# rhasspy/larynx

Measured on AMD Instinct MI355X. Metric: utterances_per_sec, higher is better.
Workload: dtype f32; 1 GPU; en-us ljspeech GlowTTS + hifi_gan 'high', batch=1, 120 phoneme ids per utterance (~623 frames = 7.24 s audio), seeded random weights, device RNG noise, fused one-call entry (mi355tts_synthesize), denoiser off (the Python API default); ids_per_utterance=120, parallelism=utterance-dp1, batch=1, calls_in_flight_per_gpu=8

## Files before the change

### larynx_amd/csrc/host_launch.h

```cpp
#pragma once

struct RowLen {
  const int* len;
  int len_const;
  template <class Args>
  void into(Args& a) const { a.len = len; a.len_const = len_const; }
};
static inline RowLen row_len(int B, int host_len, const int* dev_len, int mul = 1, int dev_const = 0) {
  if (B == 1 && host_len >= 0) return {nullptr, host_len * mul};
  return {dev_len, dev_const};
}

template <int K, int CI_C, int MB, int NB, int WN, int KS, int HALO, int EPI>
static void launch_conv_inst(ProfScope& ps, hipStream_t s, dim3 grid, const ConvArgs& a) {
  ps.kernel(KN_CONV_MFMA, a.rows);
  hipLaunchKernelGGL(HIP_KERNEL_NAME(conv_mfma_kernel<K, CI_C, MB, NB, WN, KS, HALO, EPI>), grid, dim3(64 * WN * KS), 0, s, a);
}

enum TileShape { TILE_SMALL = 0, TILE_W128 = 1, TILE_NB2 = 2, TILE_TINY = 3, TILE_LAST = 3, TILE_M128 = 4 };

static bool rb_plane_ok(const ConvArgs& a) { return (long long)a.Cin * a.x_ld < (1LL << 30); }

template <int K, int EPI>
static int launch_conv_k(ProfScope& ps, hipStream_t s, int MB, int shape, dim3 grid, const ConvArgs& a, bool rb_conv) {
  constexpr int HALO = conv_halo(K);
  constexpr int CI_SMALL = (K == 1) ? 64 : 32;
  constexpr bool PAIRED = (EPI == EPI_GATE || EPI == EPI_COUPLING);
  if (!halo_fits(K, a.dil, a.pad, HALO))
    return fail(MI355TTS_ERR_INVALID, "conv K=%d dilation=%d exceeds the staged halo", K, a.dil);
  if (a.x_ld % 4) return fail(MI355TTS_ERR_INVALID, "internal: activation row stride %d is not a multiple of 4", a.x_ld);
  if constexpr (EPI == EPI_LINEAR && K >= 3) {
    if (shape == TILE_M128) {
      ps.kernel(KN_CONV_M128, a.rows);
      hipLaunchKernelGGL(HIP_KERNEL_NAME(conv_mfma_kernel<K, 16, 1, 2, 1, 1, HALO, EPI, 4>), grid, dim3(256), 0, s, a);
      return 0;
    }
  }
  if constexpr (EPI == EPI_UPSAMPLE) {
    if (shape == TILE_M128) {
      if constexpr (K == 2) {
        if (rb_conv && a.Cin % 16 == 0 && !a.res && !a.accum && a.alpha == 1.0f && rb_plane_ok(a)) {
          if (a.x2 && a.x3) hipLaunchKernelGGL(HIP_KERNEL_NAME(rb_conv_kernel<2, 4, EPI_UPSAMPLE, true>), grid, dim3(256), 0, s, a);
          else if (!a.x2) hipLaunchKernelGGL(HIP_KERNEL_NAME(rb_conv_kernel<2, 4, EPI_UPSAMPLE, false>), grid, dim3(256), 0, s, a);
          if ((a.x2 && a.x3) || !a.x2) {
            ps.kernel(KN_RB_CONV, a.rows);
            return 0;
          }
        }
      }
      ps.kernel(KN_CONV_M128, a.rows);
      hipLaunchKernelGGL(HIP_KERNEL_NAME(conv_mfma_kernel<K, 16, 1, 2, 1, 1, HALO, EPI, 4>), grid, dim3(256), 0, s, a);
      return 0;
    }
  }
  if (shape == TILE_M128) return fail(MI355TTS_ERR_INVALID, "internal: the 128-row tile is a ResBlock conv / upsampler shape");
  if (MB == 1) {
    if (shape == TILE_TINY) launch_conv_inst<K, 64, 1, 1, 1, 8, HALO, EPI>(ps, s, grid, a);
    else if (shape == TILE_SMALL) launch_conv_inst<K, CI_SMALL, 1, 1, 2, 4, HALO, EPI>(ps, s, grid, a);
    else if (shape == TILE_W128) launch_conv_inst<K, 32, 1, 2, 2, 4, HALO, EPI>(ps, s, grid, a);
    else launch_conv_inst<K, 16, 1, 2, 4, 2, HALO, EPI>(ps, s, grid, a);
    return 0;
  }
  if constexpr (!PAIRED) {
    if (shape == TILE_TINY) launch_conv_inst<K, 64, 2, 1, 1, 8, HALO, EPI>(ps, s, grid, a);
    else if (shape == TILE_SMALL) launch_conv_inst<K, CI_SMALL, 2, 1, 2, 4, HALO, EPI>(ps, s, grid, a);
    else if (shape == TILE_W128) return fail(MI355TTS_ERR_INVALID, "internal: the 128-column tile is one m-tile high");
    else launch_conv_inst<K, 16, 2, 2, 4, 2, HALO, EPI>(ps, s, grid, a);
    return 0;
  }
  return fail(MI355TTS_ERR_INVALID, "paired epilogues run on 32-row tiles (MB == 1)");
}

struct ConvPlan {
  ConvArgs a;
  int K = 0, MB = 1, shape = TILE_TINY, epi = EPI_LINEAR, cls = 0;
  dim3 grid;
  double flop = 0;
  bool empty = true;
  int bf16 = 0;
  int n_max = 0;
  bool pinned = false;
};

enum Bf16Cfg {
  BF_A = 0,
  BF_B = 1,
  BF_C = 2,
  BF_D = 3,
  BF_K = 4,
};
struct Bf16Tile {
  int NB, WM, WN, KS;
};
constexpr Bf16Tile BF16_TILES[5] = {{4, 4, 1, 1}, {1, 4, 1, 1}, {2, 2, 2, 1}, {1, 1, 4, 1}, {4, 4, 1, 2}};
template <class F>
static bool bf16_dispatch(int cfg, int bf16, F&& f) {
  return switch_const<BF_A, BF_B, BF_C, BF_D, BF_K>(cfg, [&](auto c) {
    if (bf16 == 3) f(c, int_c<3>{});
    else f(c, int_c<1>{});
  });
}
template <int K, int EPI>
static int launch_bf16_k(int cfg, int bf16, dim3 grid, hipStream_t s, const ConvArgs& a) {
  const bool known = bf16_dispatch(cfg, bf16, [&](auto c, auto terms) {
    constexpr Bf16Tile t = BF16_TILES[decltype(c)::value];
    hipLaunchKernelGGL(HIP_KERNEL_NAME(conv_bf16_kernel<K, 1, t.NB, t.WM, t.WN, conv_halo(K), decltype(terms)::value, t.KS, EPI>), grid,
                       dim3(64 * t.WM * t.WN * t.KS), 0, s, a);
  });
  return known ? 0 : fail(MI355TTS_ERR_INVALID, "internal: bf16 tile %d", cfg);
}

static int plan_conv(const CallOptions& o, const DevConv& c, ConvArgs a, int epi, int B, int n_max, int cls, int min_tiles, int host_len, ConvPlan* out,
                     int precision = 0) {
  out->empty = true;
  out->bf16 = 0;
  if (n_max <= 0 || B <= 0) return 0;
  auto side = [&](const int*& len, int& len_const, int mul) {
    if (!len) return;
    const RowLen r = row_len(B, host_len, len, mul, len_const);
    len = r.len; len_const = r.len_const;
// ... 8 lines not shown
  a.Cin = c.Cin;
  a.rows = c.rows;
  const bool half_on = (precision == MI355TTS_PRECISION_BF16X3 || precision == MI355TTS_PRECISION_BF16) && c.w16 && (a.x_ld % 4) == 0;
  const bool bf_linear = half_on && epi == EPI_LINEAR && !a.x2 && !a.y2 && a.split >= c.rows && a.out_act == ACT_NONE &&
                         (c.K == 3 || c.K == 5 || c.K == 7 || c.K == 11) && halo_fits(c.K, a.dil, a.pad, conv_halo(c.K));
  const bool bf_ups = half_on && !o.env.bf16_ups_off && epi == EPI_UPSAMPLE && c.K == 2 && halo_fits(2, a.dil, a.pad, conv_halo(2));
  if (bf_linear || bf_ups) {
    a.w16 = c.w16;
    a.nslab = c.nslab16;
    a.rows_major = 0;
    if (epi == EPI_UPSAMPLE) {
      const double w_bytes = (double)c.mtiles16 * c.nslab16 * c.K * 2048.0, x_bytes = (double)c.Cin * (double)n_max * 4.0 * B;
      a.rows_major = (w_bytes > x_bytes && x_bytes < 3.0e6 && c.mtiles16 >= 32) ? 1 : 0;
    }
    int cfg, rows_t, cols_t;
    if (c.mtiles16 % 4 == 0) {
      const long long tiles_a = (long long)((n_max + 127) / 128) * (c.mtiles16 / 4) * B;
      cfg = tiles_a >= 256 ? BF_A : (o.env.bf_k_off ? BF_B : BF_K);
      rows_t = 128;
      cols_t = cfg == BF_B ? 32 : 128;
    } else if (c.mtiles16 == 2) {
      cfg = BF_C;
      rows_t = 64;
      cols_t = 128;
    } else {
      cfg = BF_D;
      rows_t = 32;
      cols_t = 128;
    }
    out->a = a;
    out->K = c.K;
    out->MB = 1;
    out->shape = cfg;
    out->epi = epi;
    out->cls = cls;
    out->bf16 = precision == MI355TTS_PRECISION_BF16 ? 1 : 3;
    out->n_max = n_max;
    out->pinned = false;
    out->grid = dim3((n_max + cols_t - 1) / cols_t, (c.mtiles16 * 32) / rows_t, B);
    out->flop = 2.0 * (double)c.Cout * c.Cin * (epi == EPI_UPSAMPLE ? c.K * a.up : c.K) * (double)n_max * B;
    out->empty = false;
    return 0;
  }
  int MB = c.MB;
  int ytiles = c.mtiles / MB;
  const int rows32 = (c.rows + 31) / 32;
  auto tiles = [&](int width) { return (long long)((n_max + width - 1) / width) * (width == 128 ? rows32 : ytiles) * B; };
  const long long want = min_tiles;
  int shape = TILE_TINY;
  if (tiles(256) >= want) shape = TILE_NB2;
  else if (tiles(128) >= want) shape = TILE_W128;
  else if (tiles(64) >= want) shape = TILE_SMALL;
  bool pinned = false;
  {
    int f = o.env.force_tile;
    if (o.env.force_tile_dynamic != KNOB_UNSET) f = o.env.force_tile_dynamic;
    if (o.pin_tile >= 0) f = o.pin_tile;
    if (f >= TILE_SMALL && f <= TILE_LAST) {
      shape = f;
      pinned = true;
    }
  }
  if (shape == TILE_TINY && MB == 2 && (epi == EPI_LINEAR || epi == EPI_UPSAMPLE) && tiles(32) < 256) {
    MB = 1;
    ytiles = rows32;
  }
  {
    if (o.env.ups64 && !pinned && epi == EPI_UPSAMPLE && c.MB == 2 && rows32 == 2 && shape == TILE_W128 && tiles(64) >= 256) shape = TILE_SMALL;
  }
  if (shape == TILE_W128 && MB == 2) {
    MB = 1;
    ytiles = rows32;
  }
  {
    const bool resblock_ok = epi == EPI_LINEAR && cls == KC_RESBLOCK && c.K >= 3;
    const bool upsample_ok = epi == EPI_UPSAMPLE && !o.env.m128_ups_off && c.K >= 1 && c.K <= 3;
    if (!o.env.m128_off && !pinned && (resblock_ok || upsample_ok) && rows32 % 4 == 0 && c.rows == rows32 * 32 &&
        (long long)((n_max + 127) / 128) * (rows32 / 4) * B >= o.env.m128_min_tiles) {
      shape = TILE_M128;
      MB = 1;
      ytiles = rows32 / 4;
    }
  }
  const int T_T = shape == TILE_TINY ? 32 : (shape == TILE_SMALL || shape == TILE_M128) ? 64 : (shape == TILE_NB2 ? 256 : 128);
  {
    const double w_bytes = (double)c.mtiles * c.noct * c.K * 1024.0;
    const double x_bytes = (double)c.Cin * (double)n_max * 4.0 * B;
    a.rows_major = (w_bytes > x_bytes && x_bytes < 3.0e6 && ytiles >= 8) ? 1 : 0;
  }
  out->a = a;
  out->K = c.K;
  out->MB = MB;
  out->shape = shape;
  out->epi = epi;
  out->cls = cls;
  out->n_max = n_max;
  out->pinned = pinned;
  out->grid = dim3((n_max + T_T - 1) / T_T, ytiles, B);
  out->flop = 2.0 * (double)c.Cout * c.Cin * (epi == EPI_UPSAMPLE ? c.K * a.up : c.K) * (double)n_max * B;
  out->empty = false;
  return 0;
}

template <int EPI, int... Ks>
static int launch_conv_taps(ProfScope& ps, const ConvPlan& p, const char* unsupported, hipStream_t s, bool rb_conv) {
  int rc = 0;
  if (!switch_const<Ks...>(p.K, [&](auto k) { rc = launch_conv_k<decltype(k)::value, EPI>(ps, s, p.MB, p.shape, p.grid, p.a, rb_conv); }))
    rc = fail(MI355TTS_ERR_INVALID, unsupported, p.K);
  return rc;
}
static int run_plan(mi355tts_ctx* ctx, Worker* w, const ConvPlan& p, hipStream_t stream = nullptr) {
  if (p.empty) return 0;
  hipStream_t s = stream ? stream : w->stream;
  ProfScope ps(ctx, w, p.cls, p.flop, s);
  const bool rb_conv = w->opt.rb_conv && !w->opt.env.rb_conv_off;
  if (p.bf16) {
    ps.kernel(KN_CONV_BF16, p.a.rows);
    if (p.epi == EPI_UPSAMPLE) {
      if (p.K != 2) return fail(MI355TTS_ERR_INVALID, "bf16 upsampler needs two taps");
      return launch_bf16_k<2, EPI_UPSAMPLE>(p.shape, p.bf16, p.grid, s, p.a);
    }
    int rc = 0;
    if (!switch_const<3, 5, 7, 11>(p.K, [&](auto k) { rc = launch_bf16_k<decltype(k)::value, EPI_LINEAR>(p.shape, p.bf16, p.grid, s, p.a); }))
      rc = fail(MI355TTS_ERR_INVALID, "unsupported conv kernel size %d in bf16 mode", p.K);
    return rc;
  }
  if (p.epi == EPI_LINEAR) return launch_conv_taps<EPI_LINEAR, 1, 3, 5, 7, 11>(ps, p, "unsupported conv kernel size %d", s, rb_conv);
  if (p.epi == EPI_GATE) return launch_conv_taps<EPI_GATE, 3, 5>(ps, p, "unsupported WaveNet kernel size %d", s, rb_conv);
  if (p.epi == EPI_COUPLING) return launch_conv_taps<EPI_COUPLING, 1>(ps, p, "coupling conv must be 1x1", s, rb_conv);
  return launch_conv_taps<EPI_UPSAMPLE, 1, 2, 3>(ps, p, "unsupported upsample taps %d", s, rb_conv);
}

static int launch_conv(mi355tts_ctx* ctx, Worker* w, const DevConv& c, ConvArgs a, int epi, int B, int n_max, int cls,
                       hipStream_t stream = nullptr, int min_tiles = 1024, int host_len = -1, int precision = 0) {
  ConvPlan p;
  CHECK(plan_conv(w->opt, c, a, epi, B, n_max, cls, min_tiles, host_len, &p, precision));
  return run_plan(ctx, w, p, stream);
}

struct GroupTile {
  int shape, MB, CI_C, MBT, NB, WN, KS, WM;
};
constexpr GroupTile GROUP_TILES[6] = {{TILE_M128, 0, 16, 1, 2, 1, 1, 4}, {TILE_NB2, 2, 16, 2, 2, 4, 2, 1},  {TILE_W128, 1, 32, 1, 2, 2, 4, 1},
                                      {TILE_SMALL, 2, 32, 2, 1, 2, 4, 1}, {TILE_TINY, 1, 64, 1, 1, 1, 8, 1}, {TILE_TINY, 2, 64, 2, 1, 1, 8, 1}};
static int group_tile(int shape, int MB) {
  for (int i = 0; i < 6; ++i)
    if (GROUP_TILES[i].shape == shape && (GROUP_TILES[i].MB == MB || GROUP_TILES[i].MB == 0)) return i;
  return -1;
}
template <int K0, int K1, int K2>
static void launch_group_k(ProfScope& ps, hipStream_t s, int tile, dim3 grid, const ConvGroupArgs& g) {
  ps.kernel(KN_CONV_GROUP, g.c[0].rows);
  switch_const<0, 1, 2, 3, 4, 5>(tile, [&](auto i) {
    constexpr GroupTile t = GROUP_TILES[decltype(i)::value];
    hipLaunchKernelGGL(HIP_KERNEL_NAME(conv_group_kernel<K0, K1, K2, t.CI_C, t.MBT, t.NB, t.WN, t.KS, conv_halo(K0), conv_halo(K1), conv_halo(K2), t.WM>),
                       grid, dim3(64 * t.WM * t.WN * t.KS), 0, s, g);
  });
}
static bool rb_member_ok(const ConvArgs& a, int K) {
  const int halo = K == 11 ? RbCfg<11>::HALO : K == 7 ? RbCfg<7>::HALO : RbCfg<3>::HALO;
  return !a.x2 && !a.x3 && a.bias && a.alpha == 1.0f && !a.accum && a.out_act == ACT_NONE && a.split >= a.rows && !a.y2 &&
         a.rows % 128 == 0 && halo_fits(K, a.dil, a.pad, halo) && rb_plane_ok(a);
}

static void promote_group_plans(const CallOptions& o, ConvPlan* const* plans, int n) {
  if (n != 3 || o.env.group_promote_off || !o.group_promote) return;
  int K[3], tiles[3];
// ... 402 lines not shown
```

### larynx_amd/csrc/host_options.h

```cpp
#pragma once

constexpr int KNOB_UNSET = INT_MIN;
enum KnobWhen { PROCESS, CALL };
#define MI355TTS_ENV_KNOBS(X)                                                                                                       \
  X(sync_mode, "MI355TTS_SYNC_MODE", int, 3, PROCESS, "initial g_sync_mode: 0 hipStreamSynchronize, 1 blocking event, 2 query + sleep, 3 adaptive") \
  X(queue_policy, "MI355TTS_QUEUE_POLICY", int, 0, PROCESS, "acquire_worker: 1 = an idle hardware queue first, else the BUSIEST one (probe)") \
  X(queue_probe_off, "MI355TTS_NO_QUEUE_PROBE", bool, false, PROCESS, "no measurement of which worker streams share a hardware queue") \
  X(call_coalesce_off, "MI355TTS_NO_CALL_COALESCE", bool, false, PROCESS, "every call runs alone whatever option call_coalesce says") \
  X(selfcheck_off, "MI355TTS_NO_SELFCHECK", bool, false, PROCESS, "no dispatch-order self-check (looked at again when the check would run)") \
  X(rb_tiles, "MI355TTS_RB_TILES", int, 0, PROCESS, "workgroup target per ResBlock conv launch (<= 0: 1024)")                       \
  X(glow_tiles, "MI355TTS_GLOW_TILES", int, 0, PROCESS, "workgroup target per GlowTTS conv launch (<= 0: 1024)")                    \
  X(force_tile, "MI355TTS_FORCE_TILE", int, -1, PROCESS, "pins plan_conv's tile shape (0 .. 3): sweeps")                            \
  X(ups64, "MI355TTS_UPS64", bool, true, PROCESS, "64-row upsamplers on the 64 x 64 tile; 0 = plan_conv's shape rule (A/B runs)")   \
  X(m128_off, "MI355TTS_NO_M128", bool, false, PROCESS, "no 128-row tile at all")                                                    \
  X(m128_ups_off, "MI355TTS_NO_M128_UPS", bool, false, PROCESS, "no 128-row tile for the upsamplers")                                \
  X(rb_conv_off, "MI355TTS_NO_RB_CONV", bool, false, PROCESS, "grouped 128-row launches and upsamplers on the chunked tile, as option rb_conv = 0") \
  X(group_off, "MI355TTS_NO_GROUP", bool, false, PROCESS, "no grouped launches: neither run_group nor run_pair_group")               \
  X(group_promote_off, "MI355TTS_NO_GROUP_PROMOTE", bool, false, PROCESS, "batch-1 ResBlock steps stay on the tiles plan_conv chose") \
  X(snake_off, "MI355TTS_NO_SNAKE", bool, false, PROCESS, "grouped launches keep the longest-first order")                           \
  X(pair_fusion_off, "MI355TTS_NO_PAIR_FUSION", bool, false, PROCESS, "the 32 / 64-channel stages un-fused (every mode)")            \
  X(bf16_pair_off, "MI355TTS_NO_BF16_PAIR", bool, false, PROCESS, "the 32 / 64-channel stages un-fused in the bf16 modes")           \
  X(bf_k_off, "MI355TTS_NO_BF_K", bool, false, PROCESS, "no k-split tile in the bf16 modes")                                         \
  X(bf16_ups_off, "MI355TTS_NO_BF16_UPS", bool, false, PROCESS, "upsamplers stay f32 in the bf16 modes")                             \
  X(mrf8_off, "MI355TTS_NO_MRF8", bool, false, PROCESS, "the 8-channel stage on mrf_small_kernel instead of mrf8_kernel")            \
  X(voc_out_off, "MI355TTS_NO_VOC_OUT", bool, false, PROCESS, "the generic output tail, as option voc_out = 0")                      \
  X(gate16_off, "MI355TTS_NO_GATE16", bool, false, PROCESS, "WaveNet gate convs on the 32-row tile, as option gate16 = 0")           \
  X(gate16_max_tiles, "MI355TTS_GATE16_MAX_TILES", long long, 1LL << 40, PROCESS, "gate16 only for launches of at most this many 16-row tiles") \
  X(glow_fuse_off, "MI355TTS_NO_GLOW_FUSE", bool, false, PROCESS, "no column-owner / lin16 launches, as option glow_fuse = 0")       \
  X(lin16_off, "MI355TTS_NO_LIN16", bool, false, PROCESS, "encoder convs on the generic tiles")                                      \
  X(lin16_max_tiles, "MI355TTS_LIN16_MAX_TILES", long long, 1LL << 40, PROCESS, "lin16 only for launches of at most this many tiles") \
  X(lin16_no_k1, "MI355TTS_LIN16_NO_K1", bool, false, PROCESS, "1 x 1 convs never on lin16_kernel")                                 \
  X(lin16_no_ln, "MI355TTS_LIN16_NO_LN", bool, false, PROCESS, "LayerNorm as its own launch, never lin16_kernel's prologue")        \
  X(att_big_lds, "MI355TTS_ATT_BIG_LDS", bool, false, PROCESS, "attention always on the P <= 768 instantiation (A/B runs)")         \
  X(wn_repeat, "MI355TTS_WN_REPEAT", int, 1, PROCESS, "wn_f16_kernel launched N times (probe: it is idempotent)")                   \
  X(force_tile_dynamic, "MI355TTS_FORCE_TILE_DYNAMIC", int, KNOB_UNSET, CALL, "as MI355TTS_FORCE_TILE and ahead of it (tests)")     \
  X(m128_min_tiles, "MI355TTS_M128_MIN_TILES", long long, 256, CALL, "workgroups a launch must yield before the 128-row tile is used (tests lower it)") \
  X(group_ncu, "MI355TTS_GROUP_NCU", int, KNOB_UNSET, CALL, "CUs the dispatch-order logic assumes (unset: the device's; tests)")    \
  X(promote_max_imbalance, "MI355TTS_PROMOTE_MAX_IMBALANCE", double, 1.35, CALL, "promote_group_plans: busiest CU / mean above which a step is not promoted") \
  X(rb_nb4_min_tiles, "MI355TTS_RB_NB4_MIN_TILES", int, KNOB_UNSET, CALL, "128-column ResBlock tiles from this many, whatever the load; 0 = never (unset: run_group's load rule)") \
  X(rb_pair_min_tiles, "MI355TTS_RB_PAIR_MIN_TILES", long long, 512, CALL, "tiles of the k = 11 member from which a fused step takes the 4-wave tile (tests lower it)") \
  X(bench_ablate, "MI355TTS_BENCH_ABLATE", int, 0, CALL, "mi355tts_bench_conv1d: ConvArgs::ablate (results are wrong when set)")

struct EnvKnobs {
#define X(field, name, type, def, when, doc) type field = def;
  MI355TTS_ENV_KNOBS(X)
#undef X
};
static void parse_knob(const char* e, bool* v) { *v = std::atoi(e) != 0; }
static void parse_knob(const char* e, int* v) { *v = std::atoi(e); }
static void parse_knob(const char* e, long long* v) { *v = std::atoll(e); }
static void parse_knob(const char* e, double* v) { *v = std::atof(e); }
static void read_env_knobs(KnobWhen which, EnvKnobs* k) {
#define X(field, name, type, def, when, doc)                          \
  if (when == which)                                                  \
    if (const char* e = std::getenv(name)) parse_knob(e, &k->field);
  MI355TTS_ENV_KNOBS(X)
#undef X
}
static EnvKnobs g_env;
static std::atomic<int> g_sync_mode{3};
static void init_process_knobs() {
  static const bool once = [] {
    read_env_knobs(PROCESS, &g_env);
    g_sync_mode.store(g_env.sync_mode, std::memory_order_relaxed);
    return true;
  }();
  (void)once;
}

#ifndef MI355TTS_CALL_COALESCE_DEFAULT
#define MI355TTS_CALL_COALESCE_DEFAULT 0
#endif

struct ContextOptions {
  std::atomic<bool> serial_branches{false};
  std::atomic<bool> adaptive_schedule{false};
  std::atomic<bool> gate16{true};
  std::atomic<int> gate16_wide{512};
  std::atomic<bool> glow_fuse{true};
  std::atomic<bool> voc_out{true};
  std::atomic<bool> mrf_small{true};
  std::atomic<bool> mrf_group{true};
  std::atomic<bool> rb_conv{true};
  std::atomic<bool> rb_pair{true};
  std::atomic<bool> rb_dil{true};
  std::atomic<bool> group_promote{true};
  std::atomic<bool> group_snake{true};
  std::atomic<int> call_coalesce{MI355TTS_CALL_COALESCE_DEFAULT};
  std::atomic<int> call_coalesce_window_us{300};
};

static const struct OptionRow {
  const char* name;
  std::atomic<bool> ContextOptions::*flag;
  std::atomic<int> ContextOptions::*count;
} option_table[] = {
    {"adaptive_schedule", &ContextOptions::adaptive_schedule, nullptr},
    {"mrf_small", &ContextOptions::mrf_small, nullptr},
    {"gate16", &ContextOptions::gate16, nullptr},
    {"call_coalesce", nullptr, &ContextOptions::call_coalesce},
    {"call_coalesce_window_us", nullptr, &ContextOptions::call_coalesce_window_us},
    {"glow_fuse", &ContextOptions::glow_fuse, nullptr},
    {"mrf_group", &ContextOptions::mrf_group, nullptr},
    {"rb_conv", &ContextOptions::rb_conv, nullptr},
    {"group_snake", &ContextOptions::group_snake, nullptr},
    {"group_promote", &ContextOptions::group_promote, nullptr},
    {"rb_pair", &ContextOptions::rb_pair, nullptr},
    {"rb_dil", &ContextOptions::rb_dil, nullptr},
    {"gate16_wide", nullptr, &ContextOptions::gate16_wide},
    {"voc_out", &ContextOptions::voc_out, nullptr},
    {"serial_branches", &ContextOptions::serial_branches, nullptr},
    {"sync_mode", nullptr, nullptr},
};
static int set_context_option(ContextOptions& c, const char* name, int value) {
  for (const OptionRow& r : option_table) {
    if (std::strcmp(name, r.name) != 0) continue;
    if (r.flag) {
      c.*r.flag = value != 0;
    } else if (r.count) {
      c.*r.count = value < 0 ? 0 : value;
    } else {
      if (value < 0 || value > 3) return fail(MI355TTS_ERR_INVALID, "sync_mode %d outside [0, 3]", value);
      g_sync_mode.store(value, std::memory_order_relaxed);
    }
    return 0;
  }
  return fail(MI355TTS_ERR_INVALID, "unknown option '%s'", name);
}

struct CallOptions {
  bool glow_fuse = true, gate16 = true, rb_conv = true, rb_pair = true, rb_dil = true, group_promote = true, group_snake = true;
  bool mrf_group = true, mrf_small = true, serial_branches = false, adaptive_schedule = false, voc_out = true;
  int gate16_wide = 512;
  int pin_tile = -1;
  int ncu = 256;
  EnvKnobs env;
};
static void snapshot_options(const ContextOptions& c, int device_ncu, CallOptions* o) {
  *o = CallOptions();
  o->env = g_env;
  read_env_knobs(CALL, &o->env);
  o->ncu = o->env.group_ncu != KNOB_UNSET ? o->env.group_ncu : device_ncu;
  o->glow_fuse = c.glow_fuse.load();
  o->gate16 = c.gate16.load();
  o->gate16_wide = c.gate16_wide.load();
  o->rb_conv = c.rb_conv.load();
  o->rb_pair = c.rb_pair.load();
  o->rb_dil = c.rb_dil.load();
  o->group_promote = c.group_promote.load();
  o->group_snake = c.group_snake.load();
  o->mrf_group = c.mrf_group.load();
  o->mrf_small = c.mrf_small.load();
  o->serial_branches = c.serial_branches.load();
  o->adaptive_schedule = c.adaptive_schedule.load();
  o->voc_out = c.voc_out.load();
}
```

### larynx_amd/csrc/host_profile.h

```cpp
#pragma once

#define MI355TTS_KCLASSES(X) \
  X(KC_RESBLOCK, "conv_mfma.hifigan_resblock") X(KC_UPSAMPLE, "conv_mfma.hifigan_upsample") X(KC_VOC_IO, "conv_mfma.hifigan_pre_post") \
  X(KC_GLOW_ENC_CONV, "conv_mfma.glow_encoder") X(KC_GLOW_DEC_CONV, "conv_mfma.glow_decoder") X(KC_SMALL, "elementwise") \
  X(KC_MRF_NARROW, "mrf_small.hifigan_narrow_stage")
#define MI355TTS_KNAMES(X) \
  X(KN_CONV_MFMA, "conv_mfma_kernel") X(KN_CONV_M128, "conv_mfma_kernel.m128") X(KN_CONV_GROUP, "conv_group_kernel") X(KN_RB_CONV, "rb_conv_kernel") \
  X(KN_RB_GROUP, "rb_group_kernel") X(KN_RB_GROUP_SNAKE, "rb_group_kernel.snake") X(KN_PAIR, "resblock_pair_kernel") X(KN_PAIR_GROUP, "pair_group_kernel") \
  X(KN_RB_PAIR, "rb_pair_kernel") X(KN_RB_PAIR_GROUP, "rb_pair_group_kernel") X(KN_CONV_BF16, "conv_bf16_kernel") X(KN_CONV_BF16_GROUP, "conv_bf16_group_kernel") \
  X(KN_PAIR_BF16, "pair_bf16_kernel") X(KN_PAIR_BF16_GROUP, "pair_bf16_group_kernel") X(KN_MRF_SMALL, "mrf_small_kernel") X(KN_MRF8, "mrf8_kernel") \
  X(KN_GATE16, "gate16_kernel") X(KN_GATE16_WIDE, "gate16_kernel.wide") X(KN_LIN16, "lin16_kernel") X(KN_LIN16_LN, "lin16_kernel.ln") \
  X(KN_LIN16_WIDE, "lin16_kernel.wide") X(KN_GLOW_TAIL, "glow_tail_kernel") X(KN_OPROJ_LN, "oproj_ln_kernel") X(KN_POST_CONV, "post_conv_kernel") \
  X(KN_WAVE_OUT, "wave_out_kernel") X(KN_ATTENTION, "attention_mfma_kernel") X(KN_CONV_F16, "conv_f16_kernel") X(KN_CONV_F16_GROUP, "conv_f16_group_kernel") \
  X(KN_POST_F16, "post_f16_kernel") X(KN_PACK_OCTETS, "pack_octets_kernel") X(KN_PAIR_F16_GROUP, "pair_f16_group_kernel") X(KN_WN_F16, "wn_f16_kernel") \
  X(KN_RB_GROUP_NB4, "rb_group_kernel.nb4") X(KN_GL_MAG, "griffin_lim_mag_kernel") X(KN_GL_INIT, "griffin_lim_init_kernel") X(KN_GL_ITER, "griffin_lim_iter_kernel") \
  X(KN_GL_OUT, "griffin_lim_out_kernel") X(KN_GL_INT16, "griffin_lim_int16_kernel") X(KN_GLOW_FWD, "glow_fwd_kernel") X(KN_ALIGN_SCORE, "align_score_kernel") \
  X(KN_ALIGN_PATH, "align_path_kernel") X(KN_MEL_ANALYSIS, "mel_analysis_kernel") X(KN_ATTENTION_P768, "attention_mfma_kernel.p768") X(KN_ATTENTION_VALU, "attention_kernel") \
  X(KN_LOUD_CHUNK, "loudness_chunk_kernel") X(KN_LOUD_CARRY, "loudness_carry_kernel") X(KN_LOUD_WEIGHT, "loudness_weight_kernel") \
  X(KN_LOUD_SEGMENT, "loudness_segment_kernel") X(KN_LOUD_GATE, "loudness_gate_kernel") X(KN_LOUD_APPLY, "loudness_apply_kernel") \
  X(KN_LIM_PEAK, "limiter_peak_kernel") X(KN_LIM_REDUCE, "limiter_reduce_kernel") X(KN_LIM_HOLD, "limiter_hold_kernel") \
  X(KN_LIM_CARRY, "limiter_carry_kernel") X(KN_LIM_APPLY, "limiter_apply_kernel") X(KN_PITCH, "pitch_kernel") \
  X(KN_SHIFT_MARK, "shift_mark_kernel") X(KN_SHIFT_OLA, "shift_ola_kernel")
constexpr int KN_PINNED = 44;
#define MI355TTS_X_ID(id, str) id,
#define MI355TTS_X_STR(id, str) str,
enum KClass { MI355TTS_KCLASSES(MI355TTS_X_ID) KC_COUNT };
enum KName { MI355TTS_KNAMES(MI355TTS_X_ID) KN_COUNT };
static const char* const kclass_name[KC_COUNT] = {MI355TTS_KCLASSES(MI355TTS_X_STR)};
static const char* const kname_name[KN_COUNT] = {MI355TTS_KNAMES(MI355TTS_X_STR)};
#undef MI355TTS_X_ID
#undef MI355TTS_X_STR
static_assert(KC_COUNT == 7 && KN_COUNT == 58, "a new class or name goes at the END of its table (the JSON key order is ABI) and is counted here");

struct ProfEvent {
  hipEvent_t a, b;
  int cls;
  double flop;
  int kn, sub;
};
struct ProfAcc {
  long long launches = 0;
  double ms = 0, flop = 0;
};
struct ProfSums {
  std::atomic<bool> profiling{false};
  ProfAcc prof[KC_COUNT];
  std::map<std::pair<int, int>, ProfAcc> prof_kn[KC_COUNT];
  std::atomic<long long> kn[KN_COUNT] = {};
};
struct ProfLane {
  hipStream_t stream = nullptr;
  std::vector<ProfEvent> events;
  std::vector<std::pair<hipEvent_t, hipEvent_t>> event_pool;
  double flop_scale = 1.0;
  bool quiet = false;
  int* kn_out = nullptr;
};

struct ProfScope {
  ProfSums* sums;
  ProfLane* w;
  bool on;
  ProfEvent ev;
  hipStream_t st;
  ProfScope(ProfSums* c, ProfLane* wk, int cls, double flop, hipStream_t stream = nullptr)
      : sums(c), w(wk), on(c->profiling.load() && !wk->quiet), st(stream ? stream : wk->stream) {
    if (!on) return;
    if (!w->event_pool.empty()) {
      ev.a = w->event_pool.back().first;
      ev.b = w->event_pool.back().second;
      w->event_pool.pop_back();
    } else {
      if (hipEventCreate(&ev.a) != hipSuccess || hipEventCreate(&ev.b) != hipSuccess) {
        on = false;
        return;
      }
    }
    ev.cls = cls;
    ev.flop = flop * wk->flop_scale;
    ev.kn = -1;
    ev.sub = 0;
    hipEventRecord(ev.a, st);
  }
  ProfScope(const ProfScope&) = delete;
  void kernel(int k, int sub = 0) {
    ev.kn = k;
    ev.sub = sub;
    if (!w->quiet) sums->kn[k].fetch_add(1, std::memory_order_relaxed);
    if (w->kn_out) *w->kn_out = k;
  }
  ~ProfScope() {
    if (!on) return;
    hipEventRecord(ev.b, st);
    w->events.push_back(ev);
  }
};

static void drain_profile(ProfSums* sums, ProfLane* w, std::mutex& mu) {
  if (w->events.empty()) return;
  std::lock_guard<std::mutex> lk(mu);
  for (auto& ev : w->events) {
    float ms = 0.f;
    if (hipEventElapsedTime(&ms, ev.a, ev.b) == hipSuccess) {
      for (ProfAcc* acc : {&sums->prof[ev.cls], &sums->prof_kn[ev.cls][std::make_pair(ev.kn, ev.sub)]}) {
        acc->launches++;
        acc->ms += ms;
        acc->flop += ev.flop;
      }
    }
    w->event_pool.emplace_back(ev.a, ev.b);
  }
  w->events.clear();
}

static void profile_reset(ProfSums& p) {
// ... 71 lines not shown
```

### larynx_amd/csrc/mi355tts.hip

```cpp
#include <hip/hip_runtime.h>

#include <algorithm>
#include <time.h>
#include <sys/prctl.h>
#include <atomic>
#include <condition_variable>
#include <chrono>
#include <climits>
#include <cmath>
#include <cstdarg>
#include <cstdio>
#include <cstdlib>
#include <cstring>
#include <dlfcn.h>
#include <map>
#include <memory>
#include <mutex>
#include <string>
#include <utility>
#include <vector>

#include "../../include/mi355tts.h"
#include "conv_mfma.h"
#include "rb_conv.h"
#include "resblock_pair.h"
#include "rb_pair.h"
#include "conv_bf16.h"
#include "resblock_pair_bf16.h"
#include "mrf_small.h"
#include "gate16.h"
#include "coltile.h"
#include "voc_out.h"
#include "small_kernels.h"
#include "griffin_lim.h"
#include "mel_analysis.h"
#include "resample.h"
#include "loudness.h"
#include "limiter.h"
#include "pitch.h"
#include "shift.h"
#include "align.h"
#include "conv_f16.h"
#include "pair_f16.h"
#include "wn_f16.h"
#include "weights_pack.h"

using namespace mi355tts;
#include "host_models.h"
#include "host_options.h"
#include "host_context.h"
#include "host_call.h"
#include "host_rows.h"
#include "host_group.h"
#include "host_launch.h"
#include "hifigan_f16.h"
#include "host_load.h"

extern "C" int mi355tts_abi_version(void) { return MI355TTS_ABI_VERSION; }
extern "C" const char* mi355tts_last_error(void) { return g_err.c_str(); }

extern "C" int mi355tts_create(int device, mi355tts_ctx** out) {
  if (!out) return fail(MI355TTS_ERR_INVALID, "out is null");
  int n = 0;
  HIPCHECK(hipGetDeviceCount(&n));
  if (device < 0 || device >= n) return fail(MI355TTS_ERR_INVALID, "device %d out of range (%d visible)", device, n);
  HIPCHECK(hipSetDevice(device));
  init_process_knobs();
  mi355tts_ctx* c = new mi355tts_ctx();
  c->device = device;
  {
    hipDeviceProp_t prop;
    if (hipGetDeviceProperties(&prop, device) == hipSuccess && prop.multiProcessorCount > 0) c->ncu = prop.multiProcessorCount;
  }
  *out = c;
  return 0;
}

extern "C" void mi355tts_destroy(mi355tts_ctx* ctx) {
  if (!ctx) return;
  hipSetDevice(ctx->device);
  hipDeviceSynchronize();
  for (Worker* w : ctx->all_workers) {
    for (auto& ev : w->events) {
      hipEventDestroy(ev.a);
      hipEventDestroy(ev.b);
    }
    for (auto& p : w->event_pool) {
      hipEventDestroy(p.first);
      hipEventDestroy(p.second);
    }
    for (int i = 0; i < 2; ++i) {
      if (w->aux[i]) hipStreamDestroy(w->aux[i]);
      if (w->ev_join[i]) hipEventDestroy(w->ev_join[i]);
    }
    if (w->ev_fork) hipEventDestroy(w->ev_fork);
    if (w->arena) hipFree(w->arena);
    if (w->pinned) hipHostFree(w->pinned);
    if (w->pinned_out) hipHostFree(w->pinned_out);
    if (w->stream) hipStreamDestroy(w->stream);
    delete w;
  }
  for (auto& pe : ctx->mel_pool) hipFree(pe.first);
  if (ctx->gl_table) hipFree(ctx->gl_table);
  if (ctx->hann_periodic) hipFree(ctx->hann_periodic);
  delete ctx;
}

// ... 839 lines not shown
```

Baseline: 302.1 utterances/s.

## Add column-stationary tile kernel for two-tap upsampler convolutions

Adds a new ups_col_kernel for K=2 transposed-conv upsamplers. Each workgroup stages the whole input column slab (all Cin channels, with the MRF three-way average and leaky-relu fused in) into LDS once, then walks several 128-row output groups while streaming weights. This removes the repeated input staging across row tiles that the 128-row tile incurs. The planner picks it by default (ups_col=512) when the row-group count is small and enough workgroups remain. The trade-off is a large LDS footprint, which lowers occupancy, plus fewer workgroups per launch.

```diff
diff --git a/larynx_amd/csrc/host_launch.h b/larynx_amd/csrc/host_launch.h
--- a/larynx_amd/csrc/host_launch.h
+++ b/larynx_amd/csrc/host_launch.h
@@ -17,9 +17,36 @@
   hipLaunchKernelGGL(HIP_KERNEL_NAME(conv_mfma_kernel<K, CI_C, MB, NB, WN, KS, HALO, EPI>), grid, dim3(64 * WN * KS), 0, s, a);
 }
 
-enum TileShape { TILE_SMALL = 0, TILE_W128 = 1, TILE_NB2 = 2, TILE_TINY = 3, TILE_LAST = 3, TILE_M128 = 4 };
+enum TileShape { TILE_SMALL = 0, TILE_W128 = 1, TILE_NB2 = 2, TILE_TINY = 3, TILE_LAST = 3, TILE_M128 = 4, TILE_UPS_COL = 5 };
 
 static bool rb_plane_ok(const ConvArgs& a) { return (long long)a.Cin * a.x_ld < (1LL << 30); }
+
+struct UpsColTile {
+  int MT, NB, CINP;
+};
+#ifndef UPS_COL_WIDE_TILE
+#define UPS_COL_WIDE_TILE 2, 1
+#endif
+constexpr UpsColTile UPS_COL_TILES[2] = {{1, 2, 128}, {UPS_COL_WIDE_TILE, 256}};
+static int ups_col_cfg(int Cin) { return Cin <= UPS_COL_TILES[0].CINP ? 0 : Cin <= UPS_COL_TILES[1].CINP ? 1 : -1; }
+static bool ups_col_ok(const ConvArgs& a, int K) {
+  return K == 2 && a.dil == 1 && a.pad == 1 && (a.x_ld % 4) == 0 && ((a.x2 && a.x3) || (!a.x2 && !a.x3)) && !a.res && !a.accum && a.out_act == ACT_NONE &&
+         a.alpha == 1.0f && rb_plane_ok(a) && ups_col_cfg(a.Cin) >= 0;
+}
+struct UpsColGeom {
+  int tc, nrg;
+  long long wgs;
+};
+static UpsColGeom ups_col_geom(int Cin, int rows, int B, int n_max, int ncu) {
+  const UpsColTile t = UPS_COL_TILES[ups_col_cfg(Cin)];
+  const int tc = 32 * t.NB, col_tiles = (n_max + tc - 1) / tc;
+  const int granules = ((rows + 31) / 32 + 4 * t.MT - 1) / (4 * t.MT);
+  const long long per_group = (long long)col_tiles * B;
+  int nrg = (int)std::min<long long>(granules, std::max<long long>(1, (2LL * ncu + per_group - 1) / per_group));
+  const int gpr = (granules + nrg - 1) / nrg;
+  nrg = (granules + gpr - 1) / gpr;
+  return {tc, nrg, per_group * nrg};
+}
 
 template <int K, int EPI>
 static int launch_conv_k(ProfScope& ps, hipStream_t s, int MB, int shape, dim3 grid, const ConvArgs& a, bool rb_conv) {
@@ -36,6 +63,19 @@
       return 0;
     }
   }
+  if constexpr (EPI == EPI_UPSAMPLE && K == 2) {
+    if (shape == TILE_UPS_COL) {
+      const bool mrf = a.x2 != nullptr;
+      switch_const<0, 1>(ups_col_cfg(a.Cin), [&](auto i) {
+        constexpr UpsColTile t = UPS_COL_TILES[decltype(i)::value];
+        if (mrf) hipLaunchKernelGGL(HIP_KERNEL_NAME(ups_col_kernel<true, t.MT, t.NB, t.CINP>), grid, dim3(256), 0, s, a);
+        else hipLaunchKernelGGL(HIP_KERNEL_NAME(ups_col_kernel<false, t.MT, t.NB, t.CINP>), grid, dim3(256), 0, s, a);
+      });
+      ps.kernel(KN_UPS_COL, a.rows);
+      return 0;
+    }
+  }
+  if (shape == TILE_UPS_COL) return fail(MI355TTS_ERR_INVALID, "internal: the column-stationary tile is a two-tap upsampler shape");
   if constexpr (EPI == EPI_UPSAMPLE) {
     if (shape == TILE_M128) {
       if constexpr (K == 2) {
@@ -210,7 +250,16 @@
       ytiles = rows32 / 4;
     }
   }
-  const int T_T = shape == TILE_TINY ? 32 : (shape == TILE_SMALL || shape == TILE_M128) ? 64 : (shape == TILE_NB2 ? 256 : 128);
+  int T_T = shape == TILE_TINY ? 32 : (shape == TILE_SMALL || shape == TILE_M128) ? 64 : (shape == TILE_NB2 ? 256 : 128);
+  if (epi == EPI_UPSAMPLE && !pinned && o.ups_col > 0 && ups_col_ok(a, c.K)) {
+    const UpsColGeom g = ups_col_geom(c.Cin, c.rows, B, n_max, o.ncu);
+    if (o.ups_col == 1 || (shape == TILE_M128 && c.Cin % 16 == 0 && g.nrg < c.rows / 128 && g.wgs >= o.ups_col)) {
+      shape = TILE_UPS_COL;
+      MB = 1;
+      ytiles = g.nrg;
+      T_T = g.tc;
+    }
+  }
   {
     const double w_bytes = (double)c.mtiles * c.noct * c.K * 1024.0;
     const double x_bytes = (double)c.Cin * (double)n_max * 4.0 * B;
diff --git a/larynx_amd/csrc/host_options.h b/larynx_amd/csrc/host_options.h
--- a/larynx_amd/csrc/host_options.h
+++ b/larynx_amd/csrc/host_options.h
@@ -83,6 +83,7 @@
   std::atomic<bool> mrf_group{true};
   std::atomic<bool> rb_conv{true};
   std::atomic<bool> rb_pair{true};
+  std::atomic<int> ups_col{512};
   std::atomic<bool> rb_dil{true};
   std::atomic<bool> group_promote{true};
   std::atomic<bool> group_snake{true};
@@ -107,6 +108,7 @@
     {"group_promote", &ContextOptions::group_promote, nullptr},
     {"rb_pair", &ContextOptions::rb_pair, nullptr},
     {"rb_dil", &ContextOptions::rb_dil, nullptr},
+    {"ups_col", nullptr, &ContextOptions::ups_col},
     {"gate16_wide", nullptr, &ContextOptions::gate16_wide},
     {"voc_out", &ContextOptions::voc_out, nullptr},
     {"serial_branches", &ContextOptions::serial_branches, nullptr},
@@ -131,7 +133,7 @@
 struct CallOptions {
   bool glow_fuse = true, gate16 = true, rb_conv = true, rb_pair = true, rb_dil = true, group_promote = true, group_snake = true;
   bool mrf_group = true, mrf_small = true, serial_branches = false, adaptive_schedule = false, voc_out = true;
-  int gate16_wide = 512;
+  int gate16_wide = 512, ups_col = 512;
   int pin_tile = -1;
   int ncu = 256;
   EnvKnobs env;
@@ -147,6 +149,7 @@
   o->rb_conv = c.rb_conv.load();
   o->rb_pair = c.rb_pair.load();
   o->rb_dil = c.rb_dil.load();
+  o->ups_col = c.ups_col.load();
   o->group_promote = c.group_promote.load();
   o->group_snake = c.group_snake.load();
   o->mrf_group = c.mrf_group.load();
diff --git a/larynx_amd/csrc/host_profile.h b/larynx_amd/csrc/host_profile.h
--- a/larynx_amd/csrc/host_profile.h
+++ b/larynx_amd/csrc/host_profile.h
@@ -20,7 +20,7 @@
   X(KN_LOUD_SEGMENT, "loudness_segment_kernel") X(KN_LOUD_GATE, "loudness_gate_kernel") X(KN_LOUD_APPLY, "loudness_apply_kernel") \
   X(KN_LIM_PEAK, "limiter_peak_kernel") X(KN_LIM_REDUCE, "limiter_reduce_kernel") X(KN_LIM_HOLD, "limiter_hold_kernel") \
   X(KN_LIM_CARRY, "limiter_carry_kernel") X(KN_LIM_APPLY, "limiter_apply_kernel") X(KN_PITCH, "pitch_kernel") \
-  X(KN_SHIFT_MARK, "shift_mark_kernel") X(KN_SHIFT_OLA, "shift_ola_kernel")
+  X(KN_SHIFT_MARK, "shift_mark_kernel") X(KN_SHIFT_OLA, "shift_ola_kernel") X(KN_UPS_COL, "ups_col_kernel")
 constexpr int KN_PINNED = 44;
 #define MI355TTS_X_ID(id, str) id,
 #define MI355TTS_X_STR(id, str) str,
@@ -30,7 +30,7 @@
 static const char* const kname_name[KN_COUNT] = {MI355TTS_KNAMES(MI355TTS_X_STR)};
 #undef MI355TTS_X_ID
 #undef MI355TTS_X_STR
-static_assert(KC_COUNT == 7 && KN_COUNT == 58, "a new class or name goes at the END of its table (the JSON key order is ABI) and is counted here");
+static_assert(KC_COUNT == 7 && KN_COUNT == 59, "a new class or name goes at the END of its table (the JSON key order is ABI) and is counted here");
 
 struct ProfEvent {
   hipEvent_t a, b;
diff --git a/larynx_amd/csrc/mi355tts.hip b/larynx_amd/csrc/mi355tts.hip
--- a/larynx_amd/csrc/mi355tts.hip
+++ b/larynx_amd/csrc/mi355tts.hip
@@ -23,6 +23,7 @@
 #include "../../include/mi355tts.h"
 #include "conv_mfma.h"
 #include "rb_conv.h"
+#include "ups_col.h"
 #include "resblock_pair.h"
 #include "rb_pair.h"
 #include "conv_bf16.h"
diff --git a/larynx_amd/csrc/ups_col.h b/larynx_amd/csrc/ups_col.h
--- /dev/null
+++ b/larynx_amd/csrc/ups_col.h
@@ -0,0 +1,263 @@
+#pragma once
+#include "rb_conv.h"
+
+namespace mi355tts {
+
+template <int NB>
+constexpr int ups_col_xw() { return 32 * NB + 4; }
+template <int NB, int CINP>
+constexpr int ups_col_lds_floats() { return CINP * ups_col_xw<NB>(); }
+
+__device__ __forceinline__ void ups_col_store(const ConvArgs& a, const floatx16& acc, const float (&bb)[16], int mt, int q, int b, int lane,
+                                              int Lout) {
+  const int rbase = 4 * (lane >> 5);
+  if ((a.up & 3) == 0 && (a.up_pad & 3) == 0 && (a.y_ld & 3) == 0) {
+#pragma unroll
+    for (int g4 = 0; g4 < 4; ++g4) {
+      const int row0 = mt * 32 + 8 * g4 + rbase;
+      if (row0 >= a.rows) continue;
+      const int co = row0 / a.up;
+      const int n0 = q * a.up + (row0 - co * a.up) - a.up_pad;
+      float* dst = a.y + (long long)b * a.y_bs + (long long)co * a.y_ld + n0;
+      if (n0 >= 0 && n0 + 3 < Lout) {
+        *reinterpret_cast<float4*>(dst) = make_float4(acc[4 * g4] + bb[4 * g4], acc[4 * g4 + 1] + bb[4 * g4 + 1], acc[4 * g4 + 2] + bb[4 * g4 + 2],
+                                                      acc[4 * g4 + 3] + bb[4 * g4 + 3]);
+      } else {
+#pragma unroll
+        for (int e = 0; e < 4; ++e)
+          if (n0 + e >= 0 && n0 + e < Lout) dst[e] = acc[4 * g4 + e] + bb[4 * g4 + e];
+      }
+    }
+    return;
+  }
+  if (a.up == 2) {
+#pragma unroll
+    for (int r = 0; r < 16; r += 2) {
+      const int row = mt * 32 + acc_row(r) + rbase;
+      if (row >= a.rows) continue;
+      const int co = row >> 1;
+      const int n0 = q * 2 - a.up_pad;
+      float* dst = a.y + (long long)b * a.y_bs + (long long)co * a.y_ld + n0;
+      const float v0 = acc[r] + bb[r], v1 = acc[r + 1] + bb[r + 1];
+      if (n0 >= 0 && n0 + 1 < Lout && row + 1 < a.rows) {
+        typedef float up_float2 __attribute__((ext_vector_type(2), aligned(4)));
+        *reinterpret_cast<up_float2*>(dst) = up_float2{v0, v1};
+      } else {
+        if (n0 >= 0 && n0 < Lout) dst[0] = v0;
+        if (row + 1 < a.rows && n0 + 1 >= 0 && n0 + 1 < Lout) dst[1] = v1;
+      }
+    }
+    return;
+  }
+#pragma unroll
+  for (int r = 0; r < 16; ++r) {
+    const int row = mt * 32 + acc_row(r) + rbase;
+    if (row >= a.rows) continue;
+    const int co = row / a.up;
+    const int n = q * a.up + (row - co * a.up) - a.up_pad;
+    if (n < 0 || n >= Lout) continue;
+    a.y[(long long)b * a.y_bs + (long long)co * a.y_ld + n] = acc[r] + bb[r];
+  }
+}
+
+template <bool MRF, int MT, int NB, int CINP>
+__device__ __forceinline__ void ups_col_tile(const ConvArgs& a, const int tile_x, const int rg, const int nrg, const int b, float* __restrict__ xs) {
+  constexpr int NT = 256, K = 2, TC = 32 * NB, XW = ups_col_xw<NB>(), XW4 = XW / 4, PA = 4;
+  constexpr int NP = MRF ? 3 : 1;
+  constexpr int BE = 2;
+  constexpr int RD = 4;
+  const int tid = threadIdx.x, lane = tid & 63;
+  const int wm = __builtin_amdgcn_readfirstlane(tid >> 6);
+  const int t0 = tile_x * TC;
+  const int Lin = a.in_len ? a.in_len[b] * a.in_mul : a.in_const;
+  const int Lout = a.out_len ? a.out_len[b] * a.out_mul : a.out_const;
+  const int n_len = Lin > 0 ? Lin + (K - 1) : 0;
+  if (t0 >= n_len) return;
+
+  const int mtiles = (a.rows + 31) >> 5;
+  const int granules = (mtiles + 4 * MT - 1) / (4 * MT);
+  const int gpr = (granules + nrg - 1) / nrg;
+  const int g0 = rg * gpr;
+  auto mt_of = [&](int i) { return ((g0 + i) * 4 + wm) * MT; };
+  int nwalk = 0;
+  while (nwalk < gpr && mt_of(nwalk) < mtiles) ++nwalk;
+  const int nchunks = ((a.Cin + 7) / 8 + 1) / 2;
+  const int NS = nchunks * 2 * K;
+
+  const long long mt_bytes = (long long)a.noct * K * 1024;
+  const long long step_fwd = 4 * MT * mt_bytes - (long long)(NS - 1) * 1024, step_back = -(long long)(NS - 1) * 1024;
+  const long long m_off = mtiles > 1 ? mt_bytes : 0;
+  const int mt_first = mt_of(0) < mtiles ? mt_of(0) : (mtiles - 1) & ~(MT - 1);
+  const char* pa = reinterpret_cast<const char*>(a.w) + mt_first * mt_bytes;
+  unsigned lane16 = lane * 16;
+  int pa_i = 0, pa_left = NS;
+  float4 ar[RD][MT];
+  auto a_next = [&](int slot) {
+#pragma unroll
+    for (int m = 0; m < MT; ++m) ar[slot][m] = rb_a_load(pa + m * m_off, lane16);
+    const bool wrap = --pa_left == 0, more = pa_i + 1 < nwalk;
+    pa += wrap ? (more ? step_fwd : step_back) : 1024;
+    pa_i += (wrap && more) ? 1 : 0;
+    pa_left = wrap ? NS : pa_left;
+  };
+
+  const float slope = a.in_slope;
+  const float* xb = a.x + (long long)b * a.x_bs;
+  const float* xb2 = MRF ? a.x2 + (long long)b * a.x_bs : nullptr;
+  const float* xb3 = MRF ? a.x3 + (long long)b * a.x_bs : nullptr;
+  const int cin_last = a.Cin - 1, ld_last4 = a.x_ld - 4;
+  const int used4 = (PA - a.pad + TC + (K - 1) * a.dil + 3) >> 2;
+  const int nf4 = ((a.Cin + 15) & ~15) * XW4;
+  const int nbatch = (nf4 + NT * BE - 1) / (NT * BE);
+  auto gload = [&](int batch, float4 (&pre)[BE * NP]) {
+#pragma unroll
+    for (int i = 0; i < BE; ++i) {
+      const int e = tid + NT * (batch * BE + i);
+      const int row = e / XW4, f = e - row * XW4;
+      const int rowc = row < cin_last ? row : cin_last;
+      const int c0 = t0 - PA + 4 * f;
+      unsigned off4 = (unsigned)(rowc * a.x_ld + (c0 < 0 ? 0 : (c0 > ld_last4 ? ld_last4 : c0))) * 4u;
+      pre[i] = rb_a_load(reinterpret_cast<const char*>(xb), off4);
+      if constexpr (MRF) {
+        pre[BE + i] = rb_a_load(reinterpret_cast<const char*>(xb2), off4);
+        pre[2 * BE + i] = rb_a_load(reinterpret_cast<const char*>(xb3), off4);
+      }
+    }
+  };
+  auto lstore = [&](int batch, const float4 (&pre)[BE * NP]) {
+#pragma unroll
+    for (int i = 0; i < BE; ++i) {
+      const int e = tid + NT * (batch * BE + i);
+      if (e >= nf4) continue;
+      const int row = e / XW4, f = e - row * XW4;
+      const int c0 = t0 - PA + 4 * f;
+      const bool fok = row < a.Cin && f < used4;
+      float4 v = pre[i];
+      if constexpr (MRF) {
+        const float4 v2 = pre[BE + i], v3 = pre[2 * BE + i];
+        v.x = ((v.x + v2.x) + v3.x) / a.in_div;
+        v.y = ((v.y + v2.y) + v3.y) / a.in_div;
+        v.z = ((v.z + v2.z) + v3.z) / a.in_div;
+        v.w = ((v.w + v2.w) + v3.w) / a.in_div;
+      }
+      v.x = (fok && c0 >= 0 && c0 < Lin) ? v.x : 0.f;
+      v.y = (fok && c0 + 1 >= 0 && c0 + 1 < Lin) ? v.y : 0.f;
+      v.z = (fok && c0 + 2 >= 0 && c0 + 2 < Lin) ? v.z : 0.f;
+      v.w = (fok && c0 + 3 >= 0 && c0 + 3 < Lin) ? v.w : 0.f;
+      v.x = v.x > 0.f ? v.x : v.x * slope;
+      v.y = v.y > 0.f ? v.y : v.y * slope;
+      v.z = v.z > 0.f ? v.z : v.z * slope;
+      v.w = v.w > 0.f ? v.w : v.w * slope;
+      reinterpret_cast<float4*>(xs)[e] = v;
+    }
+  };
+
+  if (RB_PRIO) __builtin_amdgcn_s_setprio(RB_PRIO);
+#pragma unroll
+  for (int s = 0; s < RD - 1; ++s) a_next(s);
+  {
+    float4 p0[BE * NP], p1[BE * NP];
+    gload(0, p0);
+    gload(1, p1);
+#pragma unroll 1
+    for (int batch = 0; batch < nbatch; batch += 2) {
+      lstore(batch, p0);
+      gload(batch + 2, p0);
+      lstore(batch + 1, p1);
+      gload(batch + 3, p1);
+    }
+  }
+  __syncthreads();
+  if (RB_PRIO) __builtin_amdgcn_s_setprio(0);
+  if (nwalk == 0) return;
+
+  const float* bp = xs + (lane >> 5) * XW + (lane & 31) + (PA - 1);
+  float bcur[4][NB], bnxt[4][NB];
+#pragma unroll
+  for (int j = 0; j < 4; ++j)
+#pragma unroll
+    for (int nb = 0; nb < NB; ++nb) bcur[j][nb] = bp[(2 * j) * XW + nb * 32];
+
+#pragma unroll 1
+  for (int i = 0; i < nwalk; ++i) {
+    floatx16 acc[MT][NB];
+#pragma unroll
+    for (int m = 0; m < MT; ++m)
+#pragma unroll
+      for (int nb = 0; nb < NB; ++nb)
+#pragma unroll
+        for (int r = 0; r < 16; ++r) acc[m][nb][r] = 0.f;
+
+#pragma unroll 1
+    for (int chunk = 0; chunk < nchunks; ++chunk) {
+      const float* xo = bp + chunk * (16 * XW);
+      const float* xn = chunk + 1 < nchunks ? xo + 16 * XW : bp;
+#pragma unroll
+      for (int s = 0; s < RD; ++s) {
+        a_next((s + RD - 1) % RD);
+        {
+          const float* src = s + 1 < RD ? xo + ((s + 1) / K) * (8 * XW) + (s + 1) % K : xn;
+#pragma unroll
+          for (int j = 0; j < 4; ++j)
+#pragma unroll
+            for (int nb = 0; nb < NB; ++nb) bnxt[j][nb] = src[(2 * j) * XW + nb * 32];
+        }
+        if constexpr (MT * NB == 1) __builtin_amdgcn_sched_barrier(0);
+#pragma unroll
+        for (int j = 0; j < 4; ++j)
+#pragma unroll
+          for (int m = 0; m < MT; ++m) {
+            const float4 af = ar[s][m];
+            const float av = (j == 0) ? af.x : (j == 1) ? af.y : (j == 2) ? af.z : af.w;
+#pragma unroll
+            for (int nb = 0; nb < NB; ++nb) acc[m][nb] = __builtin_amdgcn_mfma_f32_32x32x2f32(av, bcur[j][nb], acc[m][nb], 0, 0, 0);
+          }
+        if constexpr (MT * NB >= 2) {
+#pragma unroll
+          for (int q = 0; q < 4 * MT * NB; ++q) {
+            __builtin_amdgcn_sched_group_barrier(0x008, 1, 0);
+            if (q < MT) __builtin_amdgcn_sched_group_barrier(0x020, 1, 0);
+            else if (q < MT + 2 * NB) __builtin_amdgcn_sched_group_barrier(0x100, 1, 0);
+          }
+        }
+        __builtin_amdgcn_sched_barrier(0);
+#pragma unroll
+        for (int j = 0; j < 4; ++j)
+#pragma unroll
+          for (int nb = 0; nb < NB; ++nb) bcur[j][nb] = bnxt[j][nb];
+      }
+    }
+
+    if (RB_PRIO) __builtin_amdgcn_s_setprio(RB_PRIO);
+#pragma unroll
+    for (int m = 0; m < MT; ++m) {
+      const int mt = mt_of(i) + m;
+      if (mt >= mtiles) continue;
+      float bb[16];
+#pragma unroll
+      for (int r = 0; r < 16; ++r) bb[r] = a.bias ? a.bias[mt * 32 + acc_row(r) + 4 * (lane >> 5)] : 0.f;
+#pragma unroll
+      for (int nb = 0; nb < NB; ++nb) {
+        const int q = t0 + nb * 32 + (lane & 31);
+        if (q < n_len) ups_col_store(a, acc[m][nb], bb, mt, q, b, lane, Lout);
+      }
+    }
+    if (RB_PRIO) __builtin_amdgcn_s_setprio(0);
+  }
+}
+
+template <bool MRF, int MT, int NB, int CINP>
+__global__ __launch_bounds__(256, (160 * 1024) / (ups_col_lds_floats<NB, CINP>() * 4) >= 4 ? 4 : 2) void ups_col_kernel(const ConvArgs a) {
+  __shared__ float xs[ups_col_lds_floats<NB, CINP>()];
+  int tile_x, rg;
+  int gx = gridDim.x;
+  const int lin = blockIdx.x + blockIdx.y * gridDim.x;
+  if (gridDim.z > 1) {
+    gx = row_tiles(conv_n_len<2, EPI_UPSAMPLE>(a, blockIdx.z), 32 * NB);
+    if (lin >= gx * (int)gridDim.y) return;
+  }
+  xcd_tile_lin(lin, gx, gridDim.y, tile_x, rg, a.rows_major);
+  ups_col_tile<MRF, MT, NB, CINP>(a, tile_x, rg, gridDim.y, blockIdx.z, xs);
+}
+
+}
```

Result: no change. 302.0 utterances/s (-0.1%).
